# ultralytics/yolov3

Measured on AMD Instinct MI355X. Metric: images/sec (640x640) inference+NMS, higher is better.
Workload: dtype f16; 1 GPU; yolov3 inference 640x640 batch=32/GPU fp16 nc=80 + NMS(conf 0.001, iou 0.6, multi_label, max_det 300) [BASELINE configs[1]]; global_batch=32, parallelism=replicas x1 (no data-path collective)

## Files before the change

### yolov3_amd/csrc/api.cpp

```cpp
#include <atomic>
#include <mutex>
#include <stdarg.h>
#include <stdio.h>
#include <stdlib.h>
#include <string.h>

#include "../../include/yolov3_hip.h"
#include "y3_knobs.h"

static thread_local char g_err[512] = "";

void y3_set_error(const char* fmt, ...) {
    va_list ap;
    va_start(ap, fmt);
    vsnprintf(g_err, sizeof(g_err), fmt, ap);
    va_end(ap);
}

extern "C" const char* y3_last_error(void) { return g_err; }
extern "C" int y3_abi_version(void) { return Y3_ABI_VERSION; }

namespace {
struct Knob {
    const char* name;
    long long def;
};
const Knob kKnobs[] = {
    {"conv", 0}, {"conv_ahead", 3}, {"bn_nt_bytes", 64ll << 20},
    {"wgrad", 0}, {"wgrad_xcd", 2}, {"dgrad_quad", 1}, {"spp_direct", 0}, {"wgrad_strip", 1}, {"conv_strip", 1},
    {"conv_v10", 1}, {"v10_mp", 0}, {"v10_blocks", 0}, {"v10_half", 2}, {"v10_ksplit", 1}, {"v10_slices", 0},
    {"v10_group", 1}, {"tile_xcd", 1}, {"conv_1x1s", 1}, {"wgrad_patch", 1}, {"wgrad_blocks", 512}, {"nms_sort", 1},
    {"decode_tile", 1}, {"nms_head", 1216},
};
constexpr int kCount = (int)(sizeof(kKnobs) / sizeof(kKnobs[0]));
static_assert(kCount == Y3K_COUNT, "kKnobs and y3_knob_id (y3_common.h) list the same knobs in the same order");
std::atomic<long long> g_val[kCount];
std::once_flag g_once;

int knob_index(const char* key) {
    for (int i = 0; i < kCount; ++i)
        if (key && !strcmp(key, kKnobs[i].name)) return i;
    return -1;
}
void load_defaults() {
    for (int i = 0; i < kCount; ++i) g_val[i].store(kKnobs[i].def, std::memory_order_relaxed);
    const char* e = getenv("Y3_TUNE");
    if (!e) return;
    char buf[512];
    strncpy(buf, e, sizeof(buf) - 1);
    buf[sizeof(buf) - 1] = 0;
    for (char* tok = strtok(buf, ",;"); tok; tok = strtok(nullptr, ",;")) {
        char* eq = strchr(tok, '=');
        if (!eq) continue;
        *eq = 0;
        const int i = knob_index(tok);
        if (i >= 0) g_val[i].store(atoll(eq + 1), std::memory_order_relaxed);
        else fprintf(stderr, "libyolov3_hip: Y3_TUNE names an unknown knob '%s'\n", tok);
    }
}
}

long long y3_knob(int id) {
    std::call_once(g_once, load_defaults);
    return (id >= 0 && id < kCount) ? g_val[id].load(std::memory_order_relaxed) : 0;
}

extern "C" int y3_tune_set(const char* key, int64_t value) {
    std::call_once(g_once, load_defaults);
    const int i = knob_index(key);
    if (i < 0) {
        y3_set_error("y3_tune_set: unknown knob '%s'", key ? key : "(null)");
        return -1;
    }
    g_val[i].store((long long)value, std::memory_order_relaxed);
    return 0;
}

extern "C" int64_t y3_tune_get(const char* key) {
    std::call_once(g_once, load_defaults);
    const int i = knob_index(key);
    if (i < 0) {
        y3_set_error("y3_tune_get: unknown knob '%s'", key ? key : "(null)");
        return INT64_MIN;
    }
    return (int64_t)g_val[i].load(std::memory_order_relaxed);
// ... 7 lines not shown
```

### yolov3_amd/csrc/detect_nms.hip

```cpp
#include "y3_common.h"

#include <rocprim/rocprim.hpp>

#include <atomic>

namespace {

template <typename T>
Y3_DEV float decode_one(float v, int o, int x, int y, float stride, float aw, float ah);

template <typename T>
__global__ __launch_bounds__(256) void decode_kernel(const T* __restrict__ head, int bs, int ny, int nx, int pitch, int na, int no, float aw0, float ah0,
                                                       float aw1, float ah1, float aw2, float ah2, float aw3, float ah3, float aw4, float ah4, float stride,
                                                       T* __restrict__ raw, T* __restrict__ z, long long row_offset, long long total_rows) {
    const int nch = na * no;
    const long long idx = (long long)blockIdx.x * 256 + threadIdx.x;
    const long long total = (long long)bs * ny * nx * nch;
    if (idx >= total) return;
    const int ch = (int)(idx % nch);
    long long t = idx / nch;
    const int x = (int)(t % nx);
    t /= nx;
    const int y = (int)(t % ny);
    const int b = (int)(t / ny);
// ... 178 lines not shown
            }
        }
        ((uint4*)nxt)[tid] = vnext;
        asm volatile("" ::: "memory");
        if (live) {
            const unsigned off = (unsigned)(a * Pno + f0);
            if (L.raw) *(vec8*)((T*)L.raw + ((long long)it.b * na * Pno + (long long)it.p0 * no) + off) = rv;
            if (want_z) *(vec8*)((T*)job.z + (it.b * zimg + (L.row_offset + (long long)it.p0) * no) + off) = zv;
        }
    };
    const int step = gridDim.x;
    int item = blockIdx.x;
    Item ic = locate(item), i0, i1 = locate(item + step);
    uint4 v0 = load(ic), v1 = load(i1);
    ((uint4*)stage[0])[tid] = v0;
    __syncthreads();
    while (item < job.items) {
        i0 = locate(item + 2 * step);
        v0 = load(i0);
        compute(ic, stage[0], stage[1], v1);
        __syncthreads();
        ic = i1;
        if ((item += step) >= job.items) break;
        i1 = locate(item + 2 * step);
        v1 = load(i1);
        compute(ic, stage[1], stage[0], v0);
        __syncthreads();
        ic = i0;
        item += step;
    }
}

constexpr int IMG_BITS = 11, ORD_BITS = 21, CLS_BITS = 12, RANK_BITS = 15;
constexpr unsigned long long KEY_UNUSED = ~0ull;

struct NmsWs {
    int* row_count;
    int* row_off;
    unsigned* img_maxabs;
    unsigned* img_total;
    unsigned* img_head;
    unsigned* img_kept;
    unsigned long long* key_a;
    unsigned long long* key_b;
    unsigned* val_a;
    unsigned* val_b;
    unsigned long long* key_c;
    unsigned* val_c;
    float4* cbox;
    float* cscore;
    int* ccls;
    float4* sbox;
    unsigned char* keep;
    void* tmp;
    size_t tmp_bytes;
    long long cap;
    int own_sort;
};

template <typename T> Y3_DEV bool gt_thr(float v, float thr_T) { return v > thr_T; }

Y3_DEV bool class_allowed(int c, const int* __restrict__ classes, int ncf) {
    if (ncf == 0) return true;
    bool ok = false;
    for (int i = 0; i < ncf; ++i) ok |= (classes[i] == c);
    return ok;
}

constexpr int NMS_ROW_BATCH = 8;
template <typename T, int MODE>
__global__ __launch_bounds__(256) void nms_candidates_kernel(const T* __restrict__ pred, int bs, int n_rows, int nc, float thr, int multi_label,
                                                               const int* __restrict__ classes, int ncf, NmsWs ws, int* __restrict__ status, int ord_shift) {
    const int lane = threadIdx.x & 63;
    const int chunks_per_img = (n_rows + 63) / 64;
    const long long wave_id = (long long)blockIdx.x * 4 + (threadIdx.x >> 6);
    if (wave_id >= (long long)bs * chunks_per_img) return;
    const int img = (int)(wave_id / chunks_per_img);
    const int r0 = (int)(wave_id % chunks_per_img) * 64;
    const int no = nc + 5;
    const T* __restrict__ base = pred + (long long)img * n_rows * no;

    const int myrow = r0 + lane;
    float obj_l = 0.0f;
    if (myrow < n_rows) obj_l = to_f32<T>(base[(long long)myrow * no + 4]);
    const bool pass_l = (myrow < n_rows) && (obj_l > thr);
    unsigned long long mask = __ballot(pass_l);
    int mycount = 0;
    int myoff = 0;
    if (MODE == 1 && myrow < n_rows) myoff = ws.row_off[(long long)img * n_rows + myrow];
    const long long img_off0 = MODE == 1 ? (long long)ws.row_off[(long long)img * n_rows] : 0;
    float maxabs = 0.0f;

    if (multi_label && nc <= 128) {
        const bool in0 = lane < nc, in1 = 64 + lane < nc;
        const bool ok0 = in0 && class_allowed(lane, classes, ncf), ok1 = in1 && class_allowed(64 + lane, classes, ncf);
        while (mask) {
            int rr[NMS_ROW_BATCH];
            float v0[NMS_ROW_BATCH], v1[NMS_ROW_BATCH], bx[NMS_ROW_BATCH][4];
#pragma unroll
            for (int q = 0; q < NMS_ROW_BATCH; ++q) {
                rr[q] = mask ? __builtin_ctzll(mask) : -1;
                mask &= mask - 1;
            }
#pragma unroll
            for (int q = 0; q < NMS_ROW_BATCH; ++q) {
                const T* __restrict__ rp = base + (long long)(r0 + (rr[q] >= 0 ? rr[q] : rr[0])) * no;
                v0[q] = to_f32<T>(rp[5 + (in0 ? lane : 0)]);
                v1[q] = to_f32<T>(rp[5 + (in1 ? 64 + lane : 0)]);
#pragma unroll
                for (int i = 0; i < 4; ++i) bx[q][i] = MODE == 1 ? to_f32<T>(rp[i]) : 0.0f;
            }
#pragma unroll
            for (int q = 0; q < NMS_ROW_BATCH; ++q) {
                if (rr[q] < 0) break;
                const int r = rr[q];
                const float obj = __shfl(obj_l, r);
                int cnt = 0, off = 0;
                float4 box = make_float4(0.f, 0.f, 0.f, 0.f);
                if (MODE == 1) {
                    off = __shfl(myoff, r);
                    const float hw = rt<T>(bx[q][2] / 2.0f), hh = rt<T>(bx[q][3] / 2.0f);
                    box = make_float4(rt<T>(bx[q][0] - hw), rt<T>(bx[q][1] - hh), rt<T>(bx[q][0] + hw), rt<T>(bx[q][1] + hh));
                }
#pragma unroll
                for (int h = 0; h < 2; ++h) {
                    if (h == 1 && nc <= 64) break;
                    const int c = h * 64 + lane;
                    const float conf = (h ? in1 : in0) ? rt<T>((h ? v1[q] : v0[q]) * obj) : 0.0f;
                    const bool ok = (h ? ok1 : ok0) && (conf > thr);
                    const unsigned long long m = __ballot(ok);
                    if (MODE == 1 && ok) {
                        const int k = cnt + __builtin_popcountll(m & ((1ull << lane) - 1ull));
                        const long long g = (long long)off + k;
                        if (g < ws.cap) {
                            const unsigned ord = (unsigned)((g - img_off0) >> ord_shift);
                            ws.cbox[g] = box;
                            ws.cscore[g] = conf;
                            ws.ccls[g] = c;
                            if (!ws.own_sort) {
                                ws.key_a[g] = ((unsigned long long)img << (32 + ORD_BITS)) | ((unsigned long long)(~__float_as_uint(conf)) << ORD_BITS) |
                                              (unsigned long long)(ord & ((1u << ORD_BITS) - 1u));
                                ws.val_a[g] = (unsigned)g;
                            }
                        } else {
                            status[0] = 1;
                        }
                    }
                    cnt += __builtin_popcountll(m);
                }
                if (MODE == 1 && cnt > 0) {
                    const float m4 = fmaxf(fmaxf(fabsf(box.x), fabsf(box.y)), fmaxf(fabsf(box.z), fabsf(box.w)));
                    maxabs = (m4 == m4) ? fmaxf(maxabs, m4) : INFINITY;
                }
                if (lane == r) mycount = cnt;
            }
        }
    }
    while (mask) {
        const int r = __builtin_ctzll(mask);
        mask &= mask - 1;
        const int row = r0 + r;
        const T* __restrict__ rp = base + (long long)row * no;
        const float obj = __shfl(obj_l, r);
        int cnt = 0;
        float4 box = make_float4(0.f, 0.f, 0.f, 0.f);
        int off = 0;
        if (MODE == 1) {
            off = __shfl(myoff, r);
            const float cx = to_f32<T>(rp[0]), cy = to_f32<T>(rp[1]);
            const float hw = rt<T>(to_f32<T>(rp[2]) / 2.0f), hh = rt<T>(to_f32<T>(rp[3]) / 2.0f);
            box = make_float4(rt<T>(cx - hw), rt<T>(cy - hh), rt<T>(cx + hw), rt<T>(cy + hh));
        }
        if (multi_label) {
            for (int c0 = 0; c0 < nc; c0 += 64) {
                const int c = c0 + lane;
                float conf = 0.0f;
                bool ok = false;
                if (c < nc) {
                    conf = rt<T>(to_f32<T>(rp[5 + c]) * obj);
                    ok = (conf > thr) && class_allowed(c, classes, ncf);
                }
                const unsigned long long m = __ballot(ok);
                if (MODE == 1 && ok) {
                    const int k = cnt + __builtin_popcountll(m & ((1ull << lane) - 1ull));
                    const long long g = (long long)off + k;
                    if (g < ws.cap) {
                        const unsigned ord = (unsigned)((g - img_off0) >> ord_shift);
                        ws.cbox[g] = box;
                        ws.cscore[g] = conf;
                        ws.ccls[g] = c;
                        if (!ws.own_sort) {
                            ws.key_a[g] = ((unsigned long long)img << (32 + ORD_BITS)) | ((unsigned long long)(~__float_as_uint(conf)) << ORD_BITS) |
                                          (unsigned long long)(ord & ((1u << ORD_BITS) - 1u));
                            ws.val_a[g] = (unsigned)g;
                        }
                    } else {
                        status[0] = 1;
                    }
                }
                cnt += __builtin_popcountll(m);
            }
        } else {
            float best = -INFINITY;
            int bi = 0x7fffffff;
            for (int c = lane; c < nc; c += 64) {
                const float conf = rt<T>(to_f32<T>(rp[5 + c]) * obj);
                if (conf > best) { best = conf; bi = c; }
            }
#pragma unroll
            for (int s = 32; s >= 1; s >>= 1) {
                const float ob = __shfl_xor(best, s);
                const int oi = __shfl_xor(bi, s);
                if (ob > best || (ob == best && oi < bi)) { best = ob; bi = oi; }
            }
            const bool ok = (best > thr) && class_allowed(bi, classes, ncf);
            cnt = ok ? 1 : 0;
// ... 232 lines not shown
    const int nb = 1 << bits;
    for (int i = tid; i < nb; i += SORT_WAVES * 64) L.tot[i] = 0u;
    __syncthreads();
    for (int c0 = 0; c0 < cnt; c0 += SORT_WAVES * 64 * 4) {
        uint2 e[4];
#pragma unroll
        for (int u = 0; u < 4; ++u) {
            const int r = c0 + SORT_WAVES * 64 * u + tid;
            e[u] = load(r < cnt ? r : 0);
        }
#pragma unroll
        for (int u = 0; u < 4; ++u)
            if (c0 + SORT_WAVES * 64 * u + tid < cnt && member(e[u].x)) atomicAdd(&L.tot[digit(e[u].x)], 1u);
    }
    __syncthreads();
    if (tid < 64) {
        unsigned v[SORT_NB / 64], sum = 0;
#pragma unroll
        for (int k = 0; k < SORT_NB / 64; ++k) {
            const int d = lane * (SORT_NB / 64) + k;
            v[k] = d < nb ? L.tot[d] : 0u;
            sum += v[k];
        }
        unsigned inc = sum;
#pragma unroll
        for (int d = 1; d < 64; d <<= 1) {
            const unsigned o = __shfl_up(inc, d);
            if (lane >= d) inc += o;
        }
        unsigned run = inc - sum;
#pragma unroll
        for (int k = 0; k < SORT_NB / 64; ++k) {
            if (run < want && run + v[k] >= want) {
                L.cut[0] = (unsigned)(lane * (SORT_NB / 64) + k);
                L.cut[1] = run + v[k];
                L.cut[2] = run;
            }
            run += v[k];
        }
    }
    __syncthreads();
}

__global__ __launch_bounds__(SORT_WAVES * 64) void nms_sort_kernel(NmsWs ws, int bs, int n_rows, int max_nms, float max_wh, int agnostic, int nseg, int sbit0, int sbits,
                                                                     int n_sp, int head, int round, int max_det, int* __restrict__ status) {
    __shared__ SortLds L;
    const int img = blockIdx.x, tid = threadIdx.x;
    const long long total = ws.row_off[(long long)bs * n_rows];
    if (img == 0 && tid == 0 && round < 2) status[1] = (int)(total > 0x7fffffffLL ? 0x7fffffff : total);
    const long long start = ws.row_off[(long long)img * n_rows];
    long long cnt_ll = (long long)ws.row_off[(long long)(img + 1) * n_rows] - start;
    if (start + cnt_ll > ws.cap) cnt_ll = ws.cap - start > 0 ? ws.cap - start : 0;
    const int cnt = (int)cnt_ll;
    if (cnt <= 0) return;
    const int cntm = cnt < max_nms ? cnt : max_nms;
    if (round == 2) {
        if (ws.img_kept[img] >= (unsigned)max_det || (int)ws.img_head[img] == cntm) return;
        if (tid == 0) atomicAdd(&status[0], 2);
    }
    unsigned* const X0 = (unsigned*)ws.key_a + start, * const X1 = (unsigned*)ws.key_a + ws.cap + start;
    unsigned* const X2 = (unsigned*)ws.key_b + start, * const X3 = (unsigned*)ws.key_b + ws.cap + start;
    unsigned* const X4 = (unsigned*)ws.key_c + start, * const X5 = (unsigned*)ws.key_c + ws.cap + start;
    unsigned* const VA = ws.val_a + start, * const VB = ws.val_b + start, * const VC = ws.val_c + start;
    const float* __restrict__ score = ws.cscore + start;

    const unsigned dmask = (1u << sbits) - 1u;
    const int top = sbit0 + (n_sp - 1) * sbits;
    auto fresh = [&](int r) { return make_uint2(~__float_as_uint(score[r]), (unsigned)(start + r)); };
    unsigned cut1 = dmask, cut2 = dmask;
    int ns = cnt;
    auto top_of = [&](unsigned k) { return (k >> top) & dmask; };
    auto next_of = [&](unsigned k) { return (k >> (top - sbits)) & dmask; };
    if (round == 1 && head > 0 && cnt > head) {
        head_cutoff(L, cnt, sbits, (unsigned)head, fresh, top_of, [](unsigned) { return true; });
        cut1 = L.cut[0];
        const unsigned below = L.cut[2];
        head_cutoff(L, cnt, sbits, (unsigned)head - below, fresh, next_of, [&](unsigned k) { return top_of(k) == cut1; });
        cut2 = L.cut[0];
        ns = (int)(below + L.cut[1]);
    }
    auto in_head = [&](unsigned k) {
        const unsigned t = top_of(k);
        return t < cut1 || (t == cut1 && next_of(k) <= cut2);
    };
    for (int p = 0; p < n_sp; ++p) {
        const int shift = sbit0 + p * sbits;
        const bool last = p == n_sp - 1;
        const unsigned* kin = p == 1 ? X0 : p == 2 ? X2 : X5;
        const unsigned* vin = p == 1 ? X1 : p == 2 ? X3 : VA;
        unsigned* kout = p == 0 ? X0 : p == 1 ? X2 : X5;
        unsigned* vout = last ? VB : p == 0 ? X1 : p == 1 ? X3 : VA;
        counting_pass(
            L, p == 0 ? cnt : ns, sbits, [&](int r) { return p == 0 ? fresh(r) : make_uint2(ld_l2(kin + r), ld_l2(vin + r)); },
            [&](unsigned k) { return (k >> shift) & dmask; },
            [&](unsigned pos, unsigned k, unsigned v) {
                if (!last) kout[pos] = k;
                vout[pos] = v;
            },
            in_head);
    }

    int prep = ns < max_nms ? ns : max_nms;
    if (round == 1) {
        const int h = head < 0 ? -head : head;
        if (prep > h) prep = h;
        if (tid == 0) ws.img_head[img] = (unsigned)prep;
    }
    const bool part = !agnostic && nseg > 1 && (img_max_coord(ws, img) < max_wh * 0.5f);
    for (int r = tid; r < prep; r += SORT_WAVES * 64) {
        const unsigned g = ld_l2(VB + r);
        const float4 b = ws.cbox[g];
        const float c = (float)ws.ccls[g] * (agnostic ? 0.0f : max_wh);
        ws.sbox[start + r] = make_float4(b.x + c, b.y + c, b.z + c, b.w + c);
        ws.keep[start + r] = 0;
        if (!part) { VC[r] = (unsigned)(start + r); X4[r] = 0u; }
    }
    if (!part) return;
    int cbits = 1;
    while ((1 << cbits) < nseg) ++cbits;
    auto seg_of = [&](int r) { return make_uint2((unsigned)ws.ccls[ld_l2(VB + r)], (unsigned)(start + r)); };
    if (cbits <= 9) {
        counting_pass(L, prep, cbits, seg_of, [&](unsigned k) { return k; }, [&](unsigned pos, unsigned k, unsigned v) { X4[pos] = k; VC[pos] = v; });
    } else {
        counting_pass(L, prep, 9, seg_of, [&](unsigned k) { return k & 511u; }, [&](unsigned pos, unsigned k, unsigned v) { X0[pos] = k; X1[pos] = v; });
        counting_pass(
            L, prep, cbits - 9, [&](int r) { return make_uint2(ld_l2(X0 + r), ld_l2(X1 + r)); }, [&](unsigned k) { return k >> 9; },
            [&](unsigned pos, unsigned k, unsigned v) { X4[pos] = k; VC[pos] = v; });
    }
}

Y3_DEV long long lower_bound_u64(const unsigned long long* __restrict__ a, long long n, unsigned long long v) {
    long long lo = 0, hi = n;
    while (lo < hi) {
        const long long mid = (lo + hi) >> 1;
        if (a[mid] < v) lo = mid + 1; else hi = mid;
    }
    return lo;
}

Y3_DEV long long lower_bound_u32(const unsigned* __restrict__ a, long long n, unsigned v) {
    long long lo = 0, hi = n;
    while (lo < hi) {
        const long long mid = (lo + hi) >> 1;
        if (a[mid] < v) lo = mid + 1; else hi = mid;
    }
    return lo;
}

__global__ __launch_bounds__(256) void nms_greedy_kernel(NmsWs ws, int nseg, double iou_thr, int max_det, int max_nms, const unsigned long long* __restrict__ key2,
                                                          const unsigned* __restrict__ pos2, const unsigned* __restrict__ seg_sorted, int n_rows, int round) {
    __shared__ unsigned removed[(1 << RANK_BITS) / 32];
    __shared__ float4 blk[64];
    __shared__ unsigned long long srow[64];
    __shared__ unsigned long long s_keepm;
    __shared__ int s_kept;
    const int img = blockIdx.x / nseg, seg = blockIdx.x % nseg;
    long long lo, hi;
    if (seg_sorted) {
        const long long start = ws.row_off[(long long)img * n_rows];
        long long cnt = (long long)ws.row_off[(long long)(img + 1) * n_rows] - start;
        if (start + cnt > ws.cap) cnt = ws.cap - start > 0 ? ws.cap - start : 0;
        if (cnt > max_nms) cnt = max_nms;
        if (round == 1) cnt = ws.img_head[img];
        else if (round == 2 && (ws.img_kept[img] >= (unsigned)max_det || (long long)ws.img_head[img] == cnt)) return;
        lo = start + lower_bound_u32(seg_sorted + start, cnt, (unsigned)seg);
        hi = start + lower_bound_u32(seg_sorted + start, cnt, (unsigned)seg + 1u);
    } else {
        const unsigned long long kbase = ((unsigned long long)img << (CLS_BITS + RANK_BITS)) | ((unsigned long long)seg << RANK_BITS);
        lo = lower_bound_u64(key2, ws.cap, kbase);
        hi = lower_bound_u64(key2, ws.cap, kbase + (1ull << RANK_BITS));
    }
    const int n = (int)(hi - lo);
    if (n <= 0) return;
    const int tid = threadIdx.x, lane = tid & 63, wv = tid >> 6;
    for (int w = tid; w < 2 * ((n + 63) / 64); w += 256) removed[w] = 0u;
    if (tid == 0) s_kept = 0;
    const unsigned* __restrict__ pos = pos2 + lo;
    auto suppresses = [&](const float4 bi, const float iarea, const float4 bj) {
        const float xx1 = fmaxf(bi.x, bj.x), yy1 = fmaxf(bi.y, bj.y);
        const float xx2 = fminf(bi.z, bj.z), yy2 = fminf(bi.w, bj.w);
        float w = xx2 - xx1, h = yy2 - yy1;
        w = w > 0.0f ? w : 0.0f;
        h = h > 0.0f ? h : 0.0f;
        const float inter = w * h;
        const float jarea = (bj.z - bj.x) * (bj.w - bj.y);
        const float ovr = inter / (iarea + jarea - inter);
        return (double)ovr > iou_thr;
    };
    for (int base = 0; base < n; base += 64) {
        const int cnt = n - base < 64 ? n - base : 64;
        __syncthreads();
        const unsigned long long rem_in = (unsigned long long)removed[base >> 5] | ((unsigned long long)removed[(base >> 5) + 1] << 32);
        const unsigned long long valid = cnt == 64 ? ~0ull : ((1ull << cnt) - 1ull);
        if ((rem_in & valid) == valid) continue;
        if (tid < 64) {
            if (tid < cnt) blk[tid] = ws.sbox[pos[base + tid]];
            srow[tid] = 0ull;
        }
        __syncthreads();
        if (lane < cnt) {
            const float4 bi = blk[lane];
            const float iarea = (bi.z - bi.x) * (bi.w - bi.y);
            unsigned long long bits = 0ull;
#pragma unroll 4
            for (int q = 0; q < 16; ++q) {
                const int j = wv * 16 + q;
                if (j > lane && j < cnt && suppresses(bi, iarea, blk[j])) bits |= 1ull << j;
            }
            if (bits) atomicOr(&srow[lane], bits);
        }
        __syncthreads();
        if (wv == 0) {
            const unsigned long long row = srow[lane];
            const int row_lo = (int)(unsigned)row, row_hi = (int)(unsigned)(row >> 32);
            unsigned long long rem = rem_in, keepm = 0ull;
            int kept = s_kept;
            for (int i = 0; i < cnt && kept < max_det; ++i) {
                if (!((rem >> i) & 1ull)) {
                    keepm |= 1ull << i;
                    ++kept;
                    rem |= (unsigned long long)(unsigned)__builtin_amdgcn_readlane(row_lo, i) | ((unsigned long long)(unsigned)__builtin_amdgcn_readlane(row_hi, i) << 32);
                }
            }
            if ((keepm >> lane) & 1ull) ws.keep[pos[base + lane]] = 1;
            if (lane == 0) { s_keepm = keepm; s_kept = kept; }
        }
        __syncthreads();
        const unsigned long long keepm = s_keepm;
        if (s_kept >= max_det) break;
        if (keepm)
            for (int j = base + 64 + tid; j < n; j += 256) {
                if (removed[j >> 5] & (1u << (j & 31))) continue;
                const float4 bj = ws.sbox[pos[j]];
                unsigned long long km = keepm;
                while (km) {
                    const int i = __builtin_ctzll(km);
                    km &= km - 1ull;
                    const float4 bi = blk[i];
                    if (suppresses(bi, (bi.z - bi.x) * (bi.w - bi.y), bj)) { atomicOr(&removed[j >> 5], 1u << (j & 31)); break; }
                }
            }
    }
    if (round == 1 && tid == 0 && s_kept > 0) atomicAdd(&ws.img_kept[img], (unsigned)s_kept);
}

__global__ __launch_bounds__(256) void nms_gather_kernel(NmsWs ws, int n_rows, int max_det, int max_nms, const unsigned* __restrict__ idx1,
                                                          float* __restrict__ out_rows, int* __restrict__ out_counts, int rounds) {
    __shared__ int wave_cnt[4];
    __shared__ int s_base;
    const int img = blockIdx.x;
    const long long start = ws.row_off[(long long)img * n_rows];
    long long cnt = (long long)ws.row_off[(long long)(img + 1) * n_rows] - start;
    if (start + cnt > ws.cap) cnt = ws.cap - start > 0 ? ws.cap - start : 0;
    if (cnt > max_nms) cnt = max_nms;
    if (rounds == 2 && ws.img_kept[img] >= (unsigned)max_det) cnt = ws.img_head[img];
    const int tid = threadIdx.x, lane = tid & 63, wv = tid >> 6;
    if (tid == 0) s_base = 0;
    __syncthreads();
    for (long long c0 = 0; c0 < cnt; c0 += 256) {
        const long long i = c0 + tid;
        const bool k = (i < cnt) && ws.keep[start + i];
        const unsigned long long m = __ballot(k);
        if (lane == 0) wave_cnt[wv] = __builtin_popcountll(m);
        __syncthreads();
        int before = s_base;
        for (int w = 0; w < wv; ++w) before += wave_cnt[w];
        const int slot = before + __builtin_popcountll(m & ((1ull << lane) - 1ull));
        if (k && slot < max_det) {
            const unsigned g = idx1[start + i];
            const float4 b = ws.cbox[g];
            float* o = out_rows + ((long long)img * max_det + slot) * 6;
            o[0] = b.x; o[1] = b.y; o[2] = b.z; o[3] = b.w;
            o[4] = ws.cscore[g];
            o[5] = (float)ws.ccls[g];
        }
        __syncthreads();
        if (tid == 0) s_base += wave_cnt[0] + wave_cnt[1] + wave_cnt[2] + wave_cnt[3];
        __syncthreads();
        if (s_base >= max_det) break;
    }
    if (tid == 0) out_counts[img] = s_base < max_det ? s_base : max_det;
}

size_t align_up(size_t v) { return (v + 255) & ~(size_t)255; }

long long worst_capacity(int bs, int n_rows, int nc, const y3_nms_params* p) {
    return (long long)bs * n_rows * ((p->multi_label && nc > 1) ? nc : 1);
}
long long default_capacity(int bs, int n_rows, int nc, const y3_nms_params* p) {
    const long long worst = worst_capacity(bs, n_rows, nc, p);
    long long cap = (long long)bs * 16384;
    if (cap > worst) cap = worst;
    if (cap < 1024) cap = 1024;
    return cap;
}

size_t temp_bytes(long long cap, size_t scan_n) {
    size_t a = 0, b = 0;
    (void)rocprim::radix_sort_pairs(nullptr, a, (unsigned long long*)nullptr, (unsigned long long*)nullptr, (unsigned*)nullptr, (unsigned*)nullptr, (size_t)cap, 0u,
                                    64u, (hipStream_t)0);
    (void)rocprim::exclusive_scan(nullptr, b, (int*)nullptr, (int*)nullptr, 0, scan_n + 1, rocprim::plus<int>(), (hipStream_t)0);
    return align_up(a > b ? a : b);
}

size_t ctrl_words(int bs) { return 1 + (size_t)(64 + 64 + 1 + 1) * bs; }

size_t carve(NmsWs& ws, unsigned char* base, int bs, long long cap, size_t scan_n) {
    size_t off = 0;
    auto take = [&](size_t bytes) {
        unsigned char* p = base ? base + off : nullptr;
        off += align_up(bytes);
        return p;
    };
    ws.cap = cap;
    ws.row_count = (int*)take((scan_n + ctrl_words(bs)) * sizeof(int));
    ws.img_maxabs = ws.row_count ? (unsigned*)ws.row_count + scan_n + 1 : nullptr;
    ws.img_total = ws.img_maxabs ? ws.img_maxabs + (size_t)64 * bs : nullptr;
    ws.img_head = ws.img_maxabs ? ws.img_total + (size_t)64 * bs : nullptr;
    ws.img_kept = ws.img_maxabs ? ws.img_head + bs : nullptr;
    ws.row_off = (int*)take((scan_n + 1) * sizeof(int));
    ws.key_a = (unsigned long long*)take((size_t)cap * 8);
    ws.key_b = (unsigned long long*)take((size_t)cap * 8);
    ws.key_c = (unsigned long long*)take((size_t)cap * 8);
    ws.val_a = (unsigned*)take((size_t)cap * 4);
    ws.val_b = (unsigned*)take((size_t)cap * 4);
    ws.val_c = (unsigned*)take((size_t)cap * 4);
    ws.cbox = (float4*)take((size_t)cap * 16);
    ws.cscore = (float*)take((size_t)cap * 4);
    ws.ccls = (int*)take((size_t)cap * 4);
    ws.sbox = (float4*)take((size_t)cap * 16);
    ws.keep = (unsigned char*)take((size_t)cap);
    ws.tmp_bytes = temp_bytes(cap, scan_n);
    ws.tmp = take(ws.tmp_bytes);
    return off;
}

template <typename T>
int run_nms(const void* pred, int bs, int n_rows, int nc, const y3_nms_params* p, const int* classes, float* out_rows, int* out_counts, int* out_status,
            long long capacity, void* workspace, size_t workspace_bytes, hipStream_t st) {
    const size_t scan_n = (size_t)bs * n_rows;
    long long cap = capacity > 0 ? capacity : default_capacity(bs, n_rows, nc, p);
    const long long worst = worst_capacity(bs, n_rows, nc, p);
    if (cap > worst) cap = worst;
    if (cap < 1024) cap = 1024;
    NmsWs ws;
    const size_t need = carve(ws, nullptr, bs, cap, scan_n);
    if (need > workspace_bytes) Y3_FAIL("y3_nms: workspace too small (%zu bytes given, %zu needed for capacity %lld)", workspace_bytes, need, cap);
    if (cap > 0x7ffffff0LL) Y3_FAIL("y3_nms: capacity too large");
    carve(ws, (unsigned char*)workspace, bs, cap, scan_n);

    const float thr = (float)(T)(p->conf_thres);
    const int multi = (p->multi_label && nc > 1) ? 1 : 0;
    const int ncf = classes ? p->n_classes_filter : 0;
    int ord_shift = 0;
    while ((((long long)n_rows * (multi ? nc : 1)) >> ord_shift) >= (1ll << ORD_BITS)) ++ord_shift;
    const bool one_seg = p->agnostic != 0;
    const int nseg = one_seg ? 1 : nc;

    Y3_HIP(hipMemsetAsync(out_status, 0, 2 * sizeof(int), st));
    Y3_HIP(hipMemsetAsync(ws.row_count + scan_n, 0, ctrl_words(bs) * sizeof(int), st));
    ws.own_sort = y3_knob(Y3K_NMS_SORT) != 0 ? 1 : 0;
    if (!ws.own_sort) Y3_HIP(hipMemsetAsync(ws.key_a, 0xff, (size_t)cap * 8, st));

    const long long waves = (long long)bs * ((n_rows + 63) / 64);
    const unsigned cblocks = (unsigned)((waves + 3) / 4);
    hipLaunchKernelGGL((nms_candidates_kernel<T, 0>), dim3(cblocks), dim3(256), 0, st, (const T*)pred, bs, n_rows, nc, thr, multi, classes, ncf, ws, out_status, ord_shift);
    Y3_CHECK_LAUNCH();
    size_t tb = ws.tmp_bytes;
    if (ws.own_sort) {
        hipLaunchKernelGGL(nms_scan_kernel, dim3((unsigned)bs), dim3(1024), 0, st, ws, bs, n_rows);
        Y3_CHECK_LAUNCH();
    } else if (rocprim::exclusive_scan(ws.tmp, tb, ws.row_count, ws.row_off, 0, scan_n + 1, rocprim::plus<int>(), st) != hipSuccess) Y3_FAIL("y3_nms: scan failed");
    hipLaunchKernelGGL((nms_candidates_kernel<T, 1>), dim3(cblocks), dim3(256), 0, st, (const T*)pred, bs, n_rows, nc, thr, multi, classes, ncf, ws, out_status, ord_shift);
    Y3_CHECK_LAUNCH();
    if (ws.own_sort) {
        const bool narrow = sizeof(T) == 2;
        long long head = y3_knob(Y3K_NMS_HEAD);
        if (head > (1 << RANK_BITS)) head = 1 << RANK_BITS;
        if (head < -(1 << RANK_BITS)) head = -(1 << RANK_BITS);
        const int rounds = head != 0 ? 2 : 1;
        for (int r = rounds == 2 ? 1 : 0; r <= (rounds == 2 ? 2 : 0); ++r) {
            hipLaunchKernelGGL(nms_sort_kernel, dim3((unsigned)bs), dim3(SORT_WAVES * 64), 0, st, ws, bs, n_rows, p->max_nms, p->max_wh, p->agnostic, nseg,
                               narrow ? 13 : 0, narrow ? 9 : 8, narrow ? 2 : 4, (int)head, r, p->max_det, out_status);
            Y3_CHECK_LAUNCH();
            hipLaunchKernelGGL(nms_greedy_kernel, dim3((unsigned)(bs * nseg)), dim3(256), 0, st, ws, nseg, p->iou_thres, p->max_det, p->max_nms,
                               (const unsigned long long*)nullptr, ws.val_c, (const unsigned*)ws.key_c, n_rows, r);
            Y3_CHECK_LAUNCH();
        }
        hipLaunchKernelGGL(nms_gather_kernel, dim3((unsigned)bs), dim3(256), 0, st, ws, n_rows, p->max_det, p->max_nms, ws.val_b, out_rows, out_counts, rounds);
        Y3_CHECK_LAUNCH();
        return 0;
    }
    tb = ws.tmp_bytes;
    if (rocprim::radix_sort_pairs(ws.tmp, tb, ws.key_a, ws.key_b, ws.val_a, ws.val_b, (size_t)cap, 0u, 64u, st) != hipSuccess) Y3_FAIL("y3_nms: sort-1 failed");
    const unsigned rblocks = (unsigned)((cap + 255) / 256);
    hipLaunchKernelGGL(nms_rank_kernel, dim3(rblocks), dim3(256), 0, st, ws, bs, n_rows, p->max_nms, p->max_wh, p->agnostic, ws.key_b, ws.val_b, ws.key_a, ws.val_a,
                       out_status);
    Y3_CHECK_LAUNCH();
    tb = ws.tmp_bytes;
    if (rocprim::radix_sort_pairs(ws.tmp, tb, ws.key_a, ws.key_c, ws.val_a, ws.val_c, (size_t)cap, 0u, (unsigned)(IMG_BITS + CLS_BITS + RANK_BITS), st) != hipSuccess)
        Y3_FAIL("y3_nms: sort-2 failed");
    hipLaunchKernelGGL(nms_greedy_kernel, dim3((unsigned)(bs * nseg)), dim3(256), 0, st, ws, nseg, p->iou_thres, p->max_det, p->max_nms, ws.key_c, ws.val_c,
                       (const unsigned*)nullptr, n_rows, 0);
    Y3_CHECK_LAUNCH();
    hipLaunchKernelGGL(nms_gather_kernel, dim3((unsigned)bs), dim3(256), 0, st, ws, n_rows, p->max_det, p->max_nms, ws.val_b, out_rows, out_counts, 1);
    Y3_CHECK_LAUNCH();
    return 0;
}

}

extern "C" size_t y3_nms_workspace_bytes(int32_t bs, int32_t n_rows, int32_t nc, const y3_nms_params* p, int64_t capacity) {
    if (!p || bs <= 0 || n_rows <= 0 || nc <= 0) return 0;
    long long cap = capacity > 0 ? capacity : default_capacity(bs, n_rows, nc, p);
    const long long worst = worst_capacity(bs, n_rows, nc, p);
    if (cap > worst) cap = worst;
    if (cap < 1024) cap = 1024;
    NmsWs ws;
    return carve(ws, nullptr, bs, cap, (size_t)bs * n_rows);
}

extern "C" int y3_nms(const void* pred, int32_t dtype, int32_t bs, int32_t n_rows, int32_t nc, const y3_nms_params* p, const int32_t* classes, float* out_rows,
                      int32_t* out_counts, int32_t* out_status, int64_t capacity, void* workspace, size_t workspace_bytes, void* stream) {
    if (!pred || !p || !out_rows || !out_counts || !out_status || !workspace) Y3_FAIL("y3_nms: null argument");
    if (!(p->conf_thres >= 0.0f && p->conf_thres <= 1.0f)) Y3_FAIL("Invalid Confidence threshold %g, valid values are between 0.0 and 1.0", (double)p->conf_thres);
    if (!(p->iou_thres >= 0.0 && p->iou_thres <= 1.0)) Y3_FAIL("Invalid IoU %g, valid values are between 0.0 and 1.0", p->iou_thres);
    if (bs <= 0 || bs >= (1 << IMG_BITS) - 1) Y3_FAIL("y3_nms: batch size %d unsupported (max %d)", bs, (1 << IMG_BITS) - 2);
    if (nc <= 0 || nc >= (1 << CLS_BITS)) Y3_FAIL("y3_nms: class count %d unsupported", nc);
    if (p->max_nms <= 0 || p->max_nms > (1 << RANK_BITS) - 1) Y3_FAIL("y3_nms: max_nms %d unsupported (max %d)", p->max_nms, (1 << RANK_BITS) - 1);
    if ((long long)bs * n_rows >= 0x7fffffffLL) Y3_FAIL("y3_nms: too many rows");
    if (p->max_det <= 0) Y3_FAIL("y3_nms: max_det must be positive");
    hipStream_t st = (hipStream_t)stream;
    switch (dtype) {
        case Y3_F16: return run_nms<f16_t>(pred, bs, n_rows, nc, p, classes, out_rows, out_counts, out_status, capacity, workspace, workspace_bytes, st);
        case Y3_BF16: return run_nms<bf16_t>(pred, bs, n_rows, nc, p, classes, out_rows, out_counts, out_status, capacity, workspace, workspace_bytes, st);
        case Y3_F32: return run_nms<float>(pred, bs, n_rows, nc, p, classes, out_rows, out_counts, out_status, capacity, workspace, workspace_bytes, st);
    }
    Y3_FAIL("y3_nms: bad dtype %d", dtype);
}

namespace {
int decode_tile_sig(long long items, int cus, bool want_z) {
    const long long k = y3_knob(Y3K_DECODE_TILE);
    if (!want_z || k == 3) return 0;
    if (k == 2) return 1;
    if (k == 4) return 2;
    return items >= 4ll * cus ? 1 : 0;
}

const char* decode_tile_plan(DecodeTileJob& job, const y3_tensor* heads, int n_levels, int dtype, int na, int no, const float* anchors_px, const float* strides,
                             void* const* raws, void* z, const int64_t* row_offsets, long long total_rows) {
    if (dtype != Y3_F16 && dtype != Y3_BF16) return "not a 2-byte dtype";
    if (n_levels < 1 || n_levels > DT_MAX_LEVELS) return "more than 5 levels";
    if (no < 1) return "no < 1";
    if (z && ((uintptr_t)z & 15)) return "z is not 16-byte aligned";
    if (z && (total_rows * no) % 8) return "total_rows * no is no multiple of 8";
    const int w8 = (na * no + 7) / 8;
    int m = 8;
    while (m > 1 && (no * (m / 2)) % 8 == 0) m /= 2;
    const int tp = DT_THREADS / w8 / m * m;
    if (tp < 1) return "na * no too wide for one tile";
    memset(&job, 0, sizeof(job));
    job.z = z;
    job.total_rows = total_rows;
    job.n_levels = n_levels;
    job.bs = heads[0].n;
    job.na = na;
    job.no = no;
    job.tp = tp;
    job.w8 = w8;
    job.div_w8 = y3_make_divisor(w8);
    job.div_no = y3_make_divisor(no);
// ... 122 lines not shown
```

### yolov3_amd/csrc/y3_knobs.h

```cpp
#pragma once
enum y3_knob_id {
    Y3K_CONV = 0,
    Y3K_CONV_AHEAD,
    Y3K_BN_NT_BYTES,
    Y3K_WGRAD,
    Y3K_WGRAD_XCD,
    Y3K_DGRAD_QUAD,
    Y3K_SPP_DIRECT,
    Y3K_WGRAD_STRIP,
    Y3K_CONV_STRIP,
    Y3K_CONV_V10,
    Y3K_V10_MP,
    Y3K_V10_BLOCKS,
    Y3K_V10_HALF,
    Y3K_V10_KSPLIT,
    Y3K_V10_SLICES,
    Y3K_V10_GROUP,
    Y3K_TILE_XCD,
    Y3K_CONV_1X1S,
    Y3K_WGRAD_PATCH,
    Y3K_WGRAD_BLOCKS,
    Y3K_NMS_SORT,
    Y3K_DECODE_TILE,
    Y3K_NMS_HEAD,
    Y3K_COUNT
};
long long y3_knob(int id);
```

Baseline: 5509 images/sec.

## Reuse pass-1 row counts in NMS emit and precompute per-class segment tables

The second candidates pass now selects rows from the row counts produced by the first pass instead of re-reading and re-thresholding objectness, and loads objectness per selected row only. The sort kernel also writes a per-image, per-class segment boundary table, so the greedy NMS kernel reads lo/hi directly instead of running two binary searches per block. The table reuses the row_count buffer when it fits, which relies on row_count no longer being needed at that point. The first idea is controlled by a new knob that defaults on.

```diff
diff --git a/yolov3_amd/csrc/api.cpp b/yolov3_amd/csrc/api.cpp
--- a/yolov3_amd/csrc/api.cpp
+++ b/yolov3_amd/csrc/api.cpp
@@ -30,7 +30,7 @@
     {"wgrad", 0}, {"wgrad_xcd", 2}, {"dgrad_quad", 1}, {"spp_direct", 0}, {"wgrad_strip", 1}, {"conv_strip", 1},
     {"conv_v10", 1}, {"v10_mp", 0}, {"v10_blocks", 0}, {"v10_half", 2}, {"v10_ksplit", 1}, {"v10_slices", 0},
     {"v10_group", 1}, {"tile_xcd", 1}, {"conv_1x1s", 1}, {"wgrad_patch", 1}, {"wgrad_blocks", 512}, {"nms_sort", 1},
-    {"decode_tile", 1}, {"nms_head", 1216},
+    {"decode_tile", 1}, {"nms_head", 1216}, {"nms_emit_counts", 1},
 };
 constexpr int kCount = (int)(sizeof(kKnobs) / sizeof(kKnobs[0]));
 static_assert(kCount == Y3K_COUNT, "kKnobs and y3_knob_id (y3_common.h) list the same knobs in the same order");
diff --git a/yolov3_amd/csrc/detect_nms.hip b/yolov3_amd/csrc/detect_nms.hip
--- a/yolov3_amd/csrc/detect_nms.hip
+++ b/yolov3_amd/csrc/detect_nms.hip
@@ -254,6 +254,7 @@
     int* ccls;
     float4* sbox;
     unsigned char* keep;
+    unsigned* seg_tab;
     void* tmp;
     size_t tmp_bytes;
     long long cap;
@@ -272,7 +273,7 @@
 constexpr int NMS_ROW_BATCH = 8;
 template <typename T, int MODE>
 __global__ __launch_bounds__(256) void nms_candidates_kernel(const T* __restrict__ pred, int bs, int n_rows, int nc, float thr, int multi_label,
-                                                               const int* __restrict__ classes, int ncf, NmsWs ws, int* __restrict__ status, int ord_shift) {
+                                                               const int* __restrict__ classes, int ncf, NmsWs ws, int* __restrict__ status, int ord_shift, int from_counts) {
     const int lane = threadIdx.x & 63;
     const int chunks_per_img = (n_rows + 63) / 64;
     const long long wave_id = (long long)blockIdx.x * 4 + (threadIdx.x >> 6);
@@ -283,9 +284,15 @@
     const T* __restrict__ base = pred + (long long)img * n_rows * no;
 
     const int myrow = r0 + lane;
+    const bool by_counts = MODE == 1 && from_counts;
     float obj_l = 0.0f;
-    if (myrow < n_rows) obj_l = to_f32<T>(base[(long long)myrow * no + 4]);
-    const bool pass_l = (myrow < n_rows) && (obj_l > thr);
+    bool pass_l;
+    if (by_counts) {
+        pass_l = (myrow < n_rows) && ws.row_count[(long long)img * n_rows + myrow] > 0;
+    } else {
+        if (myrow < n_rows) obj_l = to_f32<T>(base[(long long)myrow * no + 4]);
+        pass_l = (myrow < n_rows) && (obj_l > thr);
+    }
     unsigned long long mask = __ballot(pass_l);
     int mycount = 0;
     int myoff = 0;
@@ -298,7 +305,7 @@
         const bool ok0 = in0 && class_allowed(lane, classes, ncf), ok1 = in1 && class_allowed(64 + lane, classes, ncf);
         while (mask) {
             int rr[NMS_ROW_BATCH];
-            float v0[NMS_ROW_BATCH], v1[NMS_ROW_BATCH], bx[NMS_ROW_BATCH][4];
+            float v0[NMS_ROW_BATCH], v1[NMS_ROW_BATCH], bx[NMS_ROW_BATCH][4], ob[NMS_ROW_BATCH];
 #pragma unroll
             for (int q = 0; q < NMS_ROW_BATCH; ++q) {
                 rr[q] = mask ? __builtin_ctzll(mask) : -1;
@@ -309,6 +316,7 @@
                 const T* __restrict__ rp = base + (long long)(r0 + (rr[q] >= 0 ? rr[q] : rr[0])) * no;
                 v0[q] = to_f32<T>(rp[5 + (in0 ? lane : 0)]);
                 v1[q] = to_f32<T>(rp[5 + (in1 ? 64 + lane : 0)]);
+                ob[q] = MODE == 1 ? to_f32<T>(rp[4]) : 0.0f;
 #pragma unroll
                 for (int i = 0; i < 4; ++i) bx[q][i] = MODE == 1 ? to_f32<T>(rp[i]) : 0.0f;
             }
@@ -316,7 +324,7 @@
             for (int q = 0; q < NMS_ROW_BATCH; ++q) {
                 if (rr[q] < 0) break;
                 const int r = rr[q];
-                const float obj = __shfl(obj_l, r);
+                const float obj = by_counts ? ob[q] : __shfl(obj_l, r);
                 int cnt = 0, off = 0;
                 float4 box = make_float4(0.f, 0.f, 0.f, 0.f);
                 if (MODE == 1) {
@@ -363,7 +371,7 @@
         mask &= mask - 1;
         const int row = r0 + r;
         const T* __restrict__ rp = base + (long long)row * no;
-        const float obj = __shfl(obj_l, r);
+        const float obj = by_counts ? to_f32<T>(rp[4]) : __shfl(obj_l, r);
         int cnt = 0;
         float4 box = make_float4(0.f, 0.f, 0.f, 0.f);
         int off = 0;
@@ -702,10 +710,14 @@
     long long cnt_ll = (long long)ws.row_off[(long long)(img + 1) * n_rows] - start;
     if (start + cnt_ll > ws.cap) cnt_ll = ws.cap - start > 0 ? ws.cap - start : 0;
     const int cnt = (int)cnt_ll;
-    if (cnt <= 0) return;
+    unsigned* const tab = ws.seg_tab + ((size_t)(round == 2 ? bs : 0) + img) * (nseg + 1);
+    auto flat_table = [&](unsigned first, unsigned rest) {
+        for (int s = tid; s <= nseg; s += SORT_WAVES * 64) tab[s] = s ? rest : first;
+    };
+    if (cnt <= 0) { flat_table(0u, 0u); return; }
     const int cntm = cnt < max_nms ? cnt : max_nms;
     if (round == 2) {
-        if (ws.img_kept[img] >= (unsigned)max_det || (int)ws.img_head[img] == cntm) return;
+        if (ws.img_kept[img] >= (unsigned)max_det || (int)ws.img_head[img] == cntm) { flat_table(0u, 0u); return; }
         if (tid == 0) atomicAdd(&status[0], 2);
     }
     unsigned* const X0 = (unsigned*)ws.key_a + start, * const X1 = (unsigned*)ws.key_a + ws.cap + start;
@@ -765,17 +777,24 @@
         ws.keep[start + r] = 0;
         if (!part) { VC[r] = (unsigned)(start + r); X4[r] = 0u; }
     }
-    if (!part) return;
+    if (!part) { flat_table((unsigned)start, (unsigned)(start + prep)); return; }
     int cbits = 1;
     while ((1 << cbits) < nseg) ++cbits;
     auto seg_of = [&](int r) { return make_uint2((unsigned)ws.ccls[ld_l2(VB + r)], (unsigned)(start + r)); };
     if (cbits <= 9) {
         counting_pass(L, prep, cbits, seg_of, [&](unsigned k) { return k; }, [&](unsigned pos, unsigned k, unsigned v) { X4[pos] = k; VC[pos] = v; });
+        for (int s = tid; s <= nseg; s += SORT_WAVES * 64) tab[s] = (unsigned)start + (s < nseg ? L.tot[s] : (unsigned)prep);
     } else {
         counting_pass(L, prep, 9, seg_of, [&](unsigned k) { return k & 511u; }, [&](unsigned pos, unsigned k, unsigned v) { X0[pos] = k; X1[pos] = v; });
         counting_pass(
             L, prep, cbits - 9, [&](int r) { return make_uint2(ld_l2(X0 + r), ld_l2(X1 + r)); }, [&](unsigned k) { return k >> 9; },
             [&](unsigned pos, unsigned k, unsigned v) { X4[pos] = k; VC[pos] = v; });
+        for (int r = tid; r < prep; r += SORT_WAVES * 64) {
+            const unsigned k = ld_l2(X4 + r);
+            for (unsigned s = r ? ld_l2(X4 + r - 1) + 1u : 0u; s <= k; ++s) tab[s] = (unsigned)(start + r);
+            if (r == prep - 1)
+                for (unsigned s = k + 1u; s <= (unsigned)nseg; ++s) tab[s] = (unsigned)(start + prep);
+        }
     }
 }
 
@@ -798,7 +817,7 @@
 }
 
 __global__ __launch_bounds__(256) void nms_greedy_kernel(NmsWs ws, int nseg, double iou_thr, int max_det, int max_nms, const unsigned long long* __restrict__ key2,
-                                                          const unsigned* __restrict__ pos2, const unsigned* __restrict__ seg_sorted, int n_rows, int round) {
+                                                          const unsigned* __restrict__ pos2, const unsigned* __restrict__ seg_tab, int round) {
     __shared__ unsigned removed[(1 << RANK_BITS) / 32];
     __shared__ float4 blk[64];
     __shared__ unsigned long long srow[64];
@@ -806,15 +825,10 @@
     __shared__ int s_kept;
     const int img = blockIdx.x / nseg, seg = blockIdx.x % nseg;
     long long lo, hi;
-    if (seg_sorted) {
-        const long long start = ws.row_off[(long long)img * n_rows];
-        long long cnt = (long long)ws.row_off[(long long)(img + 1) * n_rows] - start;
-        if (start + cnt > ws.cap) cnt = ws.cap - start > 0 ? ws.cap - start : 0;
-        if (cnt > max_nms) cnt = max_nms;
-        if (round == 1) cnt = ws.img_head[img];
-        else if (round == 2 && (ws.img_kept[img] >= (unsigned)max_det || (long long)ws.img_head[img] == cnt)) return;
-        lo = start + lower_bound_u32(seg_sorted + start, cnt, (unsigned)seg);
-        hi = start + lower_bound_u32(seg_sorted + start, cnt, (unsigned)seg + 1u);
+    if (seg_tab) {
+        const unsigned* t = seg_tab + ((size_t)(round == 2 ? gridDim.x / nseg : 0) + img) * (nseg + 1) + seg;
+        lo = t[0];
+        hi = t[1];
     } else {
         const unsigned long long kbase = ((unsigned long long)img << (CLS_BITS + RANK_BITS)) | ((unsigned long long)seg << RANK_BITS);
         lo = lower_bound_u64(key2, ws.cap, kbase);
@@ -823,8 +837,6 @@
     const int n = (int)(hi - lo);
     if (n <= 0) return;
     const int tid = threadIdx.x, lane = tid & 63, wv = tid >> 6;
-    for (int w = tid; w < 2 * ((n + 63) / 64); w += 256) removed[w] = 0u;
-    if (tid == 0) s_kept = 0;
     const unsigned* __restrict__ pos = pos2 + lo;
     auto suppresses = [&](const float4 bi, const float iarea, const float4 bj) {
         const float xx1 = fmaxf(bi.x, bj.x), yy1 = fmaxf(bi.y, bj.y);
@@ -837,6 +849,8 @@
         const float ovr = inter / (iarea + jarea - inter);
         return (double)ovr > iou_thr;
     };
+    for (int w = tid; w < 2 * ((n + 63) / 64); w += 256) removed[w] = 0u;
+    if (tid == 0) s_kept = 0;
     for (int base = 0; base < n; base += 64) {
         const int cnt = n - base < 64 ? n - base : 64;
         __syncthreads();
@@ -955,7 +969,7 @@
 
 size_t ctrl_words(int bs) { return 1 + (size_t)(64 + 64 + 1 + 1) * bs; }
 
-size_t carve(NmsWs& ws, unsigned char* base, int bs, long long cap, size_t scan_n) {
+size_t carve(NmsWs& ws, unsigned char* base, int bs, int nseg, long long cap, size_t scan_n) {
     size_t off = 0;
     auto take = [&](size_t bytes) {
         unsigned char* p = base ? base + off : nullptr;
@@ -982,6 +996,8 @@
     ws.keep = (unsigned char*)take((size_t)cap);
     ws.tmp_bytes = temp_bytes(cap, scan_n);
     ws.tmp = take(ws.tmp_bytes);
+    const size_t tab_words = (size_t)2 * bs * (nseg + 1);
+    ws.seg_tab = tab_words <= scan_n ? (unsigned*)ws.row_count : (unsigned*)take(tab_words * sizeof(unsigned));
     return off;
 }
 
@@ -993,19 +1009,19 @@
     const long long worst = worst_capacity(bs, n_rows, nc, p);
     if (cap > worst) cap = worst;
     if (cap < 1024) cap = 1024;
+    const bool one_seg = p->agnostic != 0;
+    const int nseg = one_seg ? 1 : nc;
     NmsWs ws;
-    const size_t need = carve(ws, nullptr, bs, cap, scan_n);
+    const size_t need = carve(ws, nullptr, bs, nseg, cap, scan_n);
     if (need > workspace_bytes) Y3_FAIL("y3_nms: workspace too small (%zu bytes given, %zu needed for capacity %lld)", workspace_bytes, need, cap);
     if (cap > 0x7ffffff0LL) Y3_FAIL("y3_nms: capacity too large");
-    carve(ws, (unsigned char*)workspace, bs, cap, scan_n);
+    carve(ws, (unsigned char*)workspace, bs, nseg, cap, scan_n);
 
     const float thr = (float)(T)(p->conf_thres);
     const int multi = (p->multi_label && nc > 1) ? 1 : 0;
     const int ncf = classes ? p->n_classes_filter : 0;
     int ord_shift = 0;
     while ((((long long)n_rows * (multi ? nc : 1)) >> ord_shift) >= (1ll << ORD_BITS)) ++ord_shift;
-    const bool one_seg = p->agnostic != 0;
-    const int nseg = one_seg ? 1 : nc;
 
     Y3_HIP(hipMemsetAsync(out_status, 0, 2 * sizeof(int), st));
     Y3_HIP(hipMemsetAsync(ws.row_count + scan_n, 0, ctrl_words(bs) * sizeof(int), st));
@@ -1014,14 +1030,15 @@
 
     const long long waves = (long long)bs * ((n_rows + 63) / 64);
     const unsigned cblocks = (unsigned)((waves + 3) / 4);
-    hipLaunchKernelGGL((nms_candidates_kernel<T, 0>), dim3(cblocks), dim3(256), 0, st, (const T*)pred, bs, n_rows, nc, thr, multi, classes, ncf, ws, out_status, ord_shift);
+    hipLaunchKernelGGL((nms_candidates_kernel<T, 0>), dim3(cblocks), dim3(256), 0, st, (const T*)pred, bs, n_rows, nc, thr, multi, classes, ncf, ws, out_status, ord_shift, 0);
     Y3_CHECK_LAUNCH();
     size_t tb = ws.tmp_bytes;
     if (ws.own_sort) {
         hipLaunchKernelGGL(nms_scan_kernel, dim3((unsigned)bs), dim3(1024), 0, st, ws, bs, n_rows);
         Y3_CHECK_LAUNCH();
     } else if (rocprim::exclusive_scan(ws.tmp, tb, ws.row_count, ws.row_off, 0, scan_n + 1, rocprim::plus<int>(), st) != hipSuccess) Y3_FAIL("y3_nms: scan failed");
-    hipLaunchKernelGGL((nms_candidates_kernel<T, 1>), dim3(cblocks), dim3(256), 0, st, (const T*)pred, bs, n_rows, nc, thr, multi, classes, ncf, ws, out_status, ord_shift);
+    hipLaunchKernelGGL((nms_candidates_kernel<T, 1>), dim3(cblocks), dim3(256), 0, st, (const T*)pred, bs, n_rows, nc, thr, multi, classes, ncf, ws, out_status, ord_shift,
+                            y3_knob(Y3K_NMS_EMIT_COUNTS) != 0 ? 1 : 0);
     Y3_CHECK_LAUNCH();
     if (ws.own_sort) {
         const bool narrow = sizeof(T) == 2;
@@ -1034,7 +1051,7 @@
                                narrow ? 13 : 0, narrow ? 9 : 8, narrow ? 2 : 4, (int)head, r, p->max_det, out_status);
             Y3_CHECK_LAUNCH();
             hipLaunchKernelGGL(nms_greedy_kernel, dim3((unsigned)(bs * nseg)), dim3(256), 0, st, ws, nseg, p->iou_thres, p->max_det, p->max_nms,
-                               (const unsigned long long*)nullptr, ws.val_c, (const unsigned*)ws.key_c, n_rows, r);
+                               (const unsigned long long*)nullptr, ws.val_c, (const unsigned*)ws.seg_tab, r);
             Y3_CHECK_LAUNCH();
         }
         hipLaunchKernelGGL(nms_gather_kernel, dim3((unsigned)bs), dim3(256), 0, st, ws, n_rows, p->max_det, p->max_nms, ws.val_b, out_rows, out_counts, rounds);
@@ -1051,7 +1068,7 @@
     if (rocprim::radix_sort_pairs(ws.tmp, tb, ws.key_a, ws.key_c, ws.val_a, ws.val_c, (size_t)cap, 0u, (unsigned)(IMG_BITS + CLS_BITS + RANK_BITS), st) != hipSuccess)
         Y3_FAIL("y3_nms: sort-2 failed");
     hipLaunchKernelGGL(nms_greedy_kernel, dim3((unsigned)(bs * nseg)), dim3(256), 0, st, ws, nseg, p->iou_thres, p->max_det, p->max_nms, ws.key_c, ws.val_c,
-                       (const unsigned*)nullptr, n_rows, 0);
+                       (const unsigned*)nullptr, 0);
     Y3_CHECK_LAUNCH();
     hipLaunchKernelGGL(nms_gather_kernel, dim3((unsigned)bs), dim3(256), 0, st, ws, n_rows, p->max_det, p->max_nms, ws.val_b, out_rows, out_counts, 1);
     Y3_CHECK_LAUNCH();
@@ -1067,7 +1084,7 @@
     if (cap > worst) cap = worst;
     if (cap < 1024) cap = 1024;
     NmsWs ws;
-    return carve(ws, nullptr, bs, cap, (size_t)bs * n_rows);
+    return carve(ws, nullptr, bs, p->agnostic ? 1 : nc, cap, (size_t)bs * n_rows);
 }
 
 extern "C" int y3_nms(const void* pred, int32_t dtype, int32_t bs, int32_t n_rows, int32_t nc, const y3_nms_params* p, const int32_t* classes, float* out_rows,
diff --git a/yolov3_amd/csrc/y3_knobs.h b/yolov3_amd/csrc/y3_knobs.h
--- a/yolov3_amd/csrc/y3_knobs.h
+++ b/yolov3_amd/csrc/y3_knobs.h
@@ -23,6 +23,7 @@
     Y3K_NMS_SORT,
     Y3K_DECODE_TILE,
     Y3K_NMS_HEAD,
+    Y3K_NMS_EMIT_COUNTS,
     Y3K_COUNT
 };
 long long y3_knob(int id);
```

Result: no change. 5504 images/sec (-0.1%).

## Replace forward suppression sweep in greedy NMS with lazy check against kept boxes

Applied to the files above, without the earlier changes.

The greedy NMS kernel no longer pushes suppression forward to every later candidate after each 64-box block, and no longer keeps a per-candidate removed bitmap in shared memory. Each new block is instead tested against the boxes kept so far, which sit in a 256-entry shared-memory list, with a global-memory fallback over the keep flags once that list fills. Work then scales with kept boxes times candidates visited rather than with all remaining candidates, and the loop can stop at max_det without having swept the tail. In exchange there are extra ballots per block and a slower overflow path that reads keep flags from global memory.

```diff
diff --git a/yolov3_amd/csrc/detect_nms.hip b/yolov3_amd/csrc/detect_nms.hip
--- a/yolov3_amd/csrc/detect_nms.hip
+++ b/yolov3_amd/csrc/detect_nms.hip
@@ -797,13 +797,14 @@
     return lo;
 }
 
+constexpr int GREEDY_KEPT_LDS = 256;
 __global__ __launch_bounds__(256) void nms_greedy_kernel(NmsWs ws, int nseg, double iou_thr, int max_det, int max_nms, const unsigned long long* __restrict__ key2,
                                                           const unsigned* __restrict__ pos2, const unsigned* __restrict__ seg_sorted, int n_rows, int round) {
-    __shared__ unsigned removed[(1 << RANK_BITS) / 32];
+    __shared__ float4 kbox[GREEDY_KEPT_LDS];
     __shared__ float4 blk[64];
     __shared__ unsigned long long srow[64];
+    __shared__ unsigned long long s_rem;
     __shared__ unsigned long long s_keepm;
-    __shared__ int s_kept;
     const int img = blockIdx.x / nseg, seg = blockIdx.x % nseg;
     long long lo, hi;
     if (seg_sorted) {
@@ -823,8 +824,7 @@
     const int n = (int)(hi - lo);
     if (n <= 0) return;
     const int tid = threadIdx.x, lane = tid & 63, wv = tid >> 6;
-    for (int w = tid; w < 2 * ((n + 63) / 64); w += 256) removed[w] = 0u;
-    if (tid == 0) s_kept = 0;
+    if (tid == 0) s_rem = 0ull;
     const unsigned* __restrict__ pos = pos2 + lo;
     auto suppresses = [&](const float4 bi, const float iarea, const float4 bj) {
         const float xx1 = fmaxf(bi.x, bj.x), yy1 = fmaxf(bi.y, bj.y);
@@ -837,20 +837,49 @@
         const float ovr = inter / (iarea + jarea - inter);
         return (double)ovr > iou_thr;
     };
+    auto area = [](const float4 b) { return (b.z - b.x) * (b.w - b.y); };
+    int kept = 0;
+    int n_lds = 0;
+    int ovf = -1;
     for (int base = 0; base < n; base += 64) {
         const int cnt = n - base < 64 ? n - base : 64;
-        __syncthreads();
-        const unsigned long long rem_in = (unsigned long long)removed[base >> 5] | ((unsigned long long)removed[(base >> 5) + 1] << 32);
         const unsigned long long valid = cnt == 64 ? ~0ull : ((1ull << cnt) - 1ull);
-        if ((rem_in & valid) == valid) continue;
-        if (tid < 64) {
-            if (tid < cnt) blk[tid] = ws.sbox[pos[base + tid]];
-            srow[tid] = 0ull;
-        }
-        __syncthreads();
-        if (lane < cnt) {
+        __syncthreads();
+        const float4 bj = ws.sbox[pos[base + (lane < cnt ? lane : 0)]];
+        if (wv == 0) {
+            if (lane < cnt) blk[lane] = bj;
+            srow[lane] = 0ull;
+        }
+        bool sup = false;
+        for (int k = wv; k < n_lds; k += 4) {
+            const float4 bi = kbox[k];
+            const bool s = suppresses(bi, area(bi), bj);
+            sup |= s;
+            if ((valid & ~__ballot(sup)) == 0ull) break;
+        }
+        if (ovf >= 0)
+            for (int c = ovf + 64 * wv; c < base; c += 256) {
+                if ((valid & ~__ballot(sup)) == 0ull) break;
+                const unsigned p = pos[c + lane];
+                const bool kf = ws.keep[p] != 0;
+                const float4 bk = kf ? ws.sbox[p] : make_float4(0.0f, 0.0f, 0.0f, 0.0f);
+                unsigned long long km = __ballot(kf);
+                while (km) {
+                    const int i = __builtin_ctzll(km);
+                    km &= km - 1ull;
+                    const float4 bi = make_float4(__shfl(bk.x, i), __shfl(bk.y, i), __shfl(bk.z, i), __shfl(bk.w, i));
+                    const bool s = suppresses(bi, area(bi), bj);
+                    sup |= s;
+                }
+            }
+        const unsigned long long mine = __ballot(sup) & valid;
+        if (lane == 0 && mine) atomicOr(&s_rem, mine);
+        __syncthreads();
+        const unsigned long long rem_in = s_rem;
+        const bool skip = (rem_in & valid) == valid;
+        if (!skip && lane < cnt) {
             const float4 bi = blk[lane];
-            const float iarea = (bi.z - bi.x) * (bi.w - bi.y);
+            const float iarea = area(bi);
             unsigned long long bits = 0ull;
 #pragma unroll 4
             for (int q = 0; q < 16; ++q) {
@@ -860,38 +889,38 @@
             if (bits) atomicOr(&srow[lane], bits);
         }
         __syncthreads();
+        if (tid == 0) s_rem = 0ull;
+        if (skip) continue;
         if (wv == 0) {
             const unsigned long long row = srow[lane];
             const int row_lo = (int)(unsigned)row, row_hi = (int)(unsigned)(row >> 32);
             unsigned long long rem = rem_in, keepm = 0ull;
-            int kept = s_kept;
-            for (int i = 0; i < cnt && kept < max_det; ++i) {
+            int k2 = kept;
+            for (int i = 0; i < cnt && k2 < max_det; ++i) {
                 if (!((rem >> i) & 1ull)) {
                     keepm |= 1ull << i;
-                    ++kept;
+                    ++k2;
                     rem |= (unsigned long long)(unsigned)__builtin_amdgcn_readlane(row_lo, i) | ((unsigned long long)(unsigned)__builtin_amdgcn_readlane(row_hi, i) << 32);
                 }
             }
             if ((keepm >> lane) & 1ull) ws.keep[pos[base + lane]] = 1;
-            if (lane == 0) { s_keepm = keepm; s_kept = kept; }
+            if (lane == 0) s_keepm = keepm;
         }
         __syncthreads();
         const unsigned long long keepm = s_keepm;
-        if (s_kept >= max_det) break;
-        if (keepm)
-            for (int j = base + 64 + tid; j < n; j += 256) {
-                if (removed[j >> 5] & (1u << (j & 31))) continue;
-                const float4 bj = ws.sbox[pos[j]];
-                unsigned long long km = keepm;
-                while (km) {
-                    const int i = __builtin_ctzll(km);
-                    km &= km - 1ull;
-                    const float4 bi = blk[i];
-                    if (suppresses(bi, (bi.z - bi.x) * (bi.w - bi.y), bj)) { atomicOr(&removed[j >> 5], 1u << (j & 31)); break; }
-                }
-            }
-    }
-    if (round == 1 && tid == 0 && s_kept > 0) atomicAdd(&ws.img_kept[img], (unsigned)s_kept);
+        const int nk = __builtin_popcountll(keepm);
+        kept += nk;
+        if (kept >= max_det) break;
+        if (ovf < 0) {
+            if (n_lds + nk <= GREEDY_KEPT_LDS) {
+                if (tid < 64 && ((keepm >> tid) & 1ull)) kbox[n_lds + __builtin_popcountll(keepm & ((1ull << tid) - 1ull))] = blk[tid];
+                n_lds += nk;
+            } else {
+                ovf = base;
+            }
+        }
+    }
+    if (round == 1 && tid == 0 && kept > 0) atomicAdd(&ws.img_kept[img], (unsigned)kept);
 }
 
 __global__ __launch_bounds__(256) void nms_gather_kernel(NmsWs ws, int n_rows, int max_det, int max_nms, const unsigned* __restrict__ idx1,
```

Measured after the change: 5363 images/sec before, 5399 images/sec after (median of 6 runs). No clear change (+0.7%).
